# openai/baselines

Hardware: NVIDIA H100
Metric: PPO2 learner env-steps/sec (higher is better)
Workload: dtype f16 operands / f32 accumulate (GAE f64 carry)

## Files before the change

### baselines_b200/csrc/conv_shift.cu

```cuda
#include <stdlib.h>

#include <type_traits>

#include "common.cuh"
#include "tc_common.cuh"

namespace b200rl {

static constexpr int SH_BM = 128;
static constexpr int SH_CONSUMER_WARPS = 8;
static constexpr int SH_TMA_WARP = SH_CONSUMER_WARPS;
__host__ __device__ constexpr int sh_threads(bool u8) { return (SH_CONSUMER_WARPS + 1) * 32 + (u8 ? 256 : 0); }
static constexpr int SH_MAX_TAPS = 16;
__host__ __device__ constexpr int sh_arows(int KH) { return KH == 1 ? 160 : 144; }
__host__ __device__ constexpr int sh_stages(int KH) { return KH == 1 ? 6 : 4; }
static constexpr int SH_U8_STAGES = 12;
static constexpr int SH_U8_WRES_BYTES = 16 * 1024;
__host__ __device__ constexpr int sh_wgrad_krows(bool u8) { return u8 ? 128 : 64; }
__host__ __device__ constexpr int sh_wres_bytes(int KH, bool u8) {
  return u8 ? SH_U8_WRES_BYTES : KH == 1 ? 80 * 1024 : 64 * 1024;
}
static constexpr int SH_BAR_BYTES = 512;
__host__ __device__ constexpr int sh_mask_stage_bytes(int BN, bool DACT) { return DACT ? SH_BM * BN / 8 : 0; }
static constexpr int SH_EPI_WARP_BYTES = 16 * 64;
static constexpr int SH_EPI_BYTES = SH_CONSUMER_WARPS * SH_EPI_WARP_BYTES;
static constexpr int SH_WROWS_K = 96;
static constexpr int SH_WABYTES = SH_WROWS_K * 128;
__host__ __device__ constexpr int sh_wgrad_qw(int BN, int KH, bool u8) { return u8 ? 2 : BN == 32 ? 4 : KH == 1 ? 3 : 2; }

static constexpr int SH_ORDER_BAR = 2;
__device__ __forceinline__ void order_wait(int wg) {
  asm volatile("bar.sync %0, %1;" ::"r"(SH_ORDER_BAR + wg), "n"(SH_CONSUMER_WARPS * 32) : "memory");
}
__device__ __forceinline__ void order_pass(int wg) {
  asm volatile("bar.arrive %0, %1;" ::"r"(SH_ORDER_BAR + 1 - wg), "n"(SH_CONSUMER_WARPS * 32) : "memory");
}

struct AddrMap {
  int mode;
  long long sN, sY, sX;
  int Cq, s;
  int Cq_log2, s_log2;
};

__device__ __forceinline__ long long map_rowbase(const AddrMap& a, int n, int y, int x) {
  if (a.mode == 2) {
    const int sm = a.s - 1;
    return (long long)n * a.sN + (long long)(y >> a.s_log2) * a.sY + (long long)(x >> a.s_log2) * a.sX +
           ((((y & sm) << a.s_log2) + (x & sm)) << a.Cq_log2);
  }
  if (a.mode == 1) return (long long)n * a.sN + ((long long)y << a.s_log2) * a.sY + ((long long)x << a.s_log2) * a.sX;
  return (long long)n * a.sN + (long long)y * a.sY + (long long)x * a.sX;
}
__device__ __forceinline__ long long map_coloff(const AddrMap& a, int col) {
  if (a.mode == 1) {
    const int cls = col >> a.Cq_log2;
    return (long long)(cls >> a.s_log2) * a.sY + (long long)(cls & (a.s - 1)) * a.sX + (col & (a.Cq - 1));
  }
  return col;
}

struct FastDiv {
  uint32_t mul, sh, d;
  __device__ __forceinline__ uint32_t div(uint32_t n) const { return __umulhi(n, mul) >> sh; }
};
static FastDiv make_fastdiv(uint32_t d) {
  FastDiv f;
  f.d = d;
  uint32_t s = 0;
  while ((1ull << s) < d) ++s;
  if (s == 0) s = 1;
  f.mul = (uint32_t)(((1ull << (31 + s)) / d) + 1);
  f.sh = s - 1;
  return f;
}

struct U8Src {
  const uint8_t* x;
  const long long* idx;
  long long sample_bytes;
  int row_bytes;
  int y_bytes, x_bytes;
  FastDiv per, wg;
};

static constexpr int U8_WARPS = 8;

__device__ __forceinline__ void u8x16_to_f16(const uint4& q, uint4& lo, uint4& hi) {
  const uint32_t w[4] = {q.x, q.y, q.z, q.w};
  uint32_t o[8];
  const __half2 k1024 = __floats2half2_rn(1024.0f, 1024.0f);
#pragma unroll
  for (int i = 0; i < 4; ++i) {
    const uint32_t a = __byte_perm(w[i], 0x64646464u, 0x5140);
    const uint32_t b = __byte_perm(w[i], 0x64646464u, 0x5342);
    const __half2 ha = __hsub2(*reinterpret_cast<const __half2*>(&a), k1024);
    const __half2 hb = __hsub2(*reinterpret_cast<const __half2*>(&b), k1024);
    o[2 * i] = *reinterpret_cast<const uint32_t*>(&ha);
    o[2 * i + 1] = *reinterpret_cast<const uint32_t*>(&hb);
  }
  lo = make_uint4(o[0], o[1], o[2], o[3]);
  hi = make_uint4(o[4], o[5], o[6], o[7]);
}


__device__ __forceinline__ uint4 ldg_stream_v4(const void* p) {
  uint4 v;
  asm volatile("ld.global.nc.L1::no_allocate.v4.u32 {%0,%1,%2,%3}, [%4];"
               : "=r"(v.x), "=r"(v.y), "=r"(v.z), "=r"(v.w)
               : "l"(p));
  return v;
}
__device__ __forceinline__ void st_shared_v4(uint32_t addr, const uint4& v) {
  asm volatile("st.shared.v4.b32 [%0], {%1,%2,%3,%4};" ::"r"(addr), "r"(v.x), "r"(v.y), "r"(v.z), "r"(v.w) : "memory");
}

template <int TR, int STAGES>
struct U8Ring {
  static constexpr int UPT = TR / 32;
  static constexpr int ROWS = STAGES * TR + 32;
  static constexpr int BYTES = ROWS * 128;
  static_assert(TR % 32 == 0 && BYTES % 1024 == 0, "ring keeps the 1024 B swizzle atoms aligned");
};

__device__ __forceinline__ long long u8_lookup(const U8Src& u, long long row_start, int unit, int total, long long M,
                                               int lane) {
  const long long m = row_start + (long long)unit * 32 + lane;
  if (unit >= total || m < 0 || m >= M) return -1;
  const uint32_t n = u.per.div((uint32_t)m);
  return u.idx ? __ldg(u.idx + n) : (long long)n;
}
__device__ __forceinline__ void u8_load(const U8Src& u, long long row_start, int unit, long long sb, int lane,
                                        uint4 (&q)[4]) {
  if (sb >= 0) {
    const uint32_t mm = (uint32_t)(row_start + (long long)unit * 32 + lane);
    const uint32_t rem = mm - u.per.div(mm) * u.per.d;
    const uint32_t Y = u.wg.div(rem), X = rem - Y * u.wg.d;
    const uint8_t* src = u.x + sb * u.sample_bytes + (long long)(Y * (uint32_t)u.y_bytes + X * (uint32_t)u.x_bytes);
#pragma unroll
    for (int dy = 0; dy < 4; ++dy) q[dy] = ldg_stream_v4(src + (long long)dy * u.row_bytes);
  } else {
#pragma unroll
    for (int dy = 0; dy < 4; ++dy) q[dy] = make_uint4(0u, 0u, 0u, 0u);
  }
}

template <int TR, int STAGES, int D>
__device__ __forceinline__ void u8_ring_producer(const U8Src& u, long long M, long long row_start, int ntiles,
                                                 uint8_t* ring, uint64_t* full_bar, uint64_t* head_bar,
                                                 uint64_t* empty_bar, int pw, int lane) {
  using R = U8Ring<TR, STAGES>;
  constexpr int UPT = R::UPT, RND = U8_WARPS * D;
  if (ntiles <= 0) return;
  const int total = ntiles * UPT + 1;
  const uint32_t ring0 = smem_u32(ring) + lane * 128 + ((lane & 7) << 4);
  uint4 q[D][4];
  long long sb[D];
#pragma unroll
  for (int d = 0; d < D; ++d) sb[d] = u8_lookup(u, row_start, pw + U8_WARPS * d, total, M, lane);
#pragma unroll
  for (int d = 0; d < D; ++d) {
    u8_load(u, row_start, pw + U8_WARPS * d, sb[d], lane, q[d]);
    sb[d] = u8_lookup(u, row_start, pw + U8_WARPS * d + RND, total, M, lane);
  }
  for (int base = pw; base < total; base += RND) {
#pragma unroll
    for (int d = 0; d < D; ++d) {
      const int uc = base + U8_WARPS * d;
      if (uc < total) {
        const int tile = uc / UPT, ub = uc - tile * UPT;
        const int s = tile % STAGES;
        const uint32_t fill = (uint32_t)(tile / STAGES);
        mbar_wait(&empty_bar[s], (fill & 1u) ^ 1u);
        const uint32_t dst = ring0 + (uint32_t)(s * TR + ub * 32) * 128u;
        const bool mirror = (s == 0) && (ub == 0);
#pragma unroll
        for (int dy = 0; dy < 4; ++dy) {
          uint4 lo, hi;
          u8x16_to_f16(q[d][dy], lo, hi);
          st_shared_v4(dst ^ (uint32_t)((2 * dy) << 4), lo);
          st_shared_v4(dst ^ (uint32_t)((2 * dy + 1) << 4), hi);
// ... 148 lines not shown
    }
  } else if (U8 && warp > SH_TMA_WARP) {
    u8_ring_producer<SH_BM, STAGES, 2>(p.u8, p.M, (long long)tile_first * SH_BM + p.min_shift, tile_count, smem,
                                       full_bar, head_bar, empty_bar, warp - (SH_TMA_WARP + 1), lane);
  } else {
    const int wg = __shfl_sync(0xffffffffu, warp >> 2, 0), t = threadIdx.x & 127;
    const int row0 = PINGPONG ? 0 : wg * 64;
    const uint32_t w_base = smem_u32(wres);
    const float lo = (p.act == ACT_RELU) ? 0.0f : -INFINITY;
    const __half2 lo2 = __floats2half2_rn(lo, lo);
    const __half2 zero2 = __floats2half2_rn(0.0f, 0.0f);
    const int er = lane & 15, ep = lane >> 4;
    const int erow = row0 + 16 * (warp & 3) + er;
    uint32_t epi_addr[2];
#pragma unroll
    for (int jj = 0; jj < 2; ++jj)
      epi_addr[jj] = smem_u32(sepi + warp * SH_EPI_WARP_BYTES) + er * 64 + (((2 * jj + ep) ^ ((er >> 1) & 3)) << 4);
    const bool masked = DACT && p.saved_bits != nullptr;
    float acc[MH][BN / 2];
    mbar_wait(w_bar, 0);
    for (int i = PINGPONG ? wg : 0; i < tile_count; i += PINGPONG ? 2 : 1) {
      const int tile = tile_first + i * tile_stride;
      const int s = i % STAGES, s1 = (s + 1 == STAGES) ? 0 : s + 1;
      const uint32_t ph = (uint32_t)(i / STAGES) & 1u;
      mbar_wait(&full_bar[s], ph);
      if (U8) mbar_wait(&head_bar[s1], s1 == 0 ? ph ^ 1 : ph);
      if (PINGPONG && i > 0) order_wait(wg);
      const uint32_t a_base = smem_u32(smem + s * A_PITCH) + (uint32_t)(row0 * 128);
      wgmma_fence();
#pragma unroll 1
      for (int a = 0; a < p.taps; ++a) {
        const uint32_t at = a_base + (uint32_t)p.shift[a] * 128u;
        const uint32_t wt = w_base + (uint32_t)(a * KH * w_sub);
#pragma unroll
        for (int h = 0; h < KH; ++h) {
#pragma unroll
          for (int k = 0; k < 4; ++k) {
            const uint64_t bdesc = make_sdesc(wt + h * w_sub + k * 32, 16, 1024, 1);
#pragma unroll
            for (int mh = 0; mh < MH; ++mh) {
              const uint64_t adesc = make_sdesc(at + mh * 64 * 128 + h * SH_ABYTES + k * 32, 16, 1024, 1);
              wgmma_f16<BN, 0, 0>(acc[mh], adesc, bdesc, (a | h | k) ? 1u : 0u);
            }
          }
        }
      }
      wgmma_commit();
      if (PINGPONG && i + 1 < tile_count) order_pass(wg);
      wgmma_wait<0>();
      auto release = [&]() {
        __syncwarp();
        if (lane == 0) {
          mbar_arrive(&empty_bar[s]);
          if (U8) mbar_arrive(&empty_bar[s1]);
        }
      };
      uint32_t mrow[MH][BN / 32];
      if (masked) {
#pragma unroll
        for (int mh = 0; mh < MH; ++mh) {
          const uint32_t r = smem_u32(smask + s * MASK_STAGE) + (uint32_t)((erow + mh * 64) * (BN / 8));
#pragma unroll
          for (int i = 0; i < BN / 32; ++i) asm volatile("ld.shared.b32 %0, [%1];" : "=r"(mrow[mh][i]) : "r"(r + 4 * i));
        }
      } else {
        release();
      }

#pragma unroll
      for (int mh = 0; mh < MH; ++mh) {
        const uint32_t m = (uint32_t)tile * SH_BM + mh * 64 + erow;
        const uint32_t t2 = p.fwg.div(m);
        const int x = (int)(m - t2 * (uint32_t)p.Wg);
        const int n = (int)p.fhg.div(t2);
        const int y = (int)(t2 - (uint32_t)n * (uint32_t)p.Hg);
        const bool ok = ((long long)m < p.M) && (y < p.vy) && (x < p.vx);
        const long long obase = map_rowbase(p.omap, n, y, x);
#pragma unroll
        for (int ps = 0; ps < BN / 32; ++ps) {
#pragma unroll
          for (int jj = 0; jj < 2; ++jj) {
            const int b = 2 * (2 * ps + jj);
            uint32_t r[4];
#pragma unroll
            for (int k = 0; k < 4; ++k) {
              const int e = 4 * (b + (k >> 1)) + 2 * (k & 1);
              const int c = 8 * (b + (k >> 1)) + 2 * (t & 3);
              __half2 o;
              if (DACT) {
                o = __floats2half2_rn(acc[mh][e] * p.alpha, acc[mh][e + 1] * p.alpha);
              } else {
                o = __hmax2(__floats2half2_rn(fmaf(acc[mh][e], p.alpha, s_bias[c]),
                                              fmaf(acc[mh][e + 1], p.alpha, s_bias[c + 1])),
                            lo2);
              }
              r[k] = h2_bits(o);
            }
            stmatrix_x4(epi_addr[jj], r);
          }
          __syncwarp();
#pragma unroll
          for (int jj = 0; jj < 2; ++jj) {
            const int j = 2 * ps + jj;
            uint4 v = ld_shared_v4(epi_addr[jj]);
            const long long ocol = map_coloff(p.omap, 16 * j);
            if (masked) {
              const uint32_t b8 = (mrow[mh][j >> 1] >> (16 * (j & 1) + 8 * ep)) & 0xffu;
              v.x &= mask_pair(b8, 0);
              v.y &= mask_pair(b8, 1);
              v.z &= mask_pair(b8, 2);
              v.w &= mask_pair(b8, 3);
            }
            if (ok) st_global_v4(p.out + obase + ocol + 8 * ep, v);
            if (!DACT && p.bits_out != nullptr) {
              const uint32_t w[4] = {v.x, v.y, v.z, v.w};
              uint32_t bits = 0;
#pragma unroll
              for (int k = 0; k < 4; ++k) {
                const uint32_t gt = __hgt2_mask(*reinterpret_cast<const __half2*>(&w[k]), zero2);
                bits |= ((gt & 1u) | ((gt >> 15) & 2u)) << (2 * k);
              }
              bits <<= 8 * ep;
              bits |= __shfl_xor_sync(0xffffffffu, bits, 16);
              if (ok && ep == 0) p.bits_out[(obase + ocol) >> 4] = (uint16_t)bits;
            }
          }
          __syncwarp();
        }
      }
      if (masked) release();
    }
  }
}

struct ShiftWgradParams {
  U8Src u8;
  float* gbias;
  float alpha_b;
  long long M;
  int N;
  int taps;
  int kx;
  int shift[SH_MAX_TAPS];
  float* G;
  long long ldg;
  float alpha;
  int kb_total, kb_per_cta;
  float* ws_g;
  float* ws_b;
  long long grows;
};

template <int BN, int KH, bool U8>
__global__ void __launch_bounds__(sh_threads(U8), 1)
conv_shift_wgrad_kernel(const __grid_constant__ CUtensorMap tmX, const __grid_constant__ CUtensorMap tmD,
                        const __grid_constant__ ShiftWgradParams p) {
  constexpr int BROWB = (BN >= 64) ? 128 : BN * 2;
  constexpr uint32_t LAYOUT_B = sdesc_layout(BROWB);
  constexpr int KR = sh_wgrad_krows(U8);
  constexpr int B_BYTES = KR * BROWB;
  constexpr int B_REGION = (B_BYTES + 1023) & ~1023;
  constexpr int STAGES = (KH == 1) ? 8 : 6;
  constexpr int QW = sh_wgrad_qw(BN, KH, U8);
  static_assert(!U8 || KH == 1, "the uint8-fed layer has 64 space-to-depth channels");
  using Ring = U8Ring<KR, STAGES>;
  constexpr int A_PITCH = U8 ? KR * 128 : KH * SH_WABYTES + B_REGION;
  constexpr int B_PITCH = U8 ? B_REGION : KH * SH_WABYTES + B_REGION;
  constexpr int B_BASE = U8 ? Ring::BYTES : KH * SH_WABYTES;
  constexpr int SMEM_TILES = U8 ? Ring::BYTES + STAGES * B_REGION : STAGES * (KH * SH_WABYTES + B_REGION);
  extern __shared__ uint8_t smem_raw[];
  uint8_t* smem = reinterpret_cast<uint8_t*>((reinterpret_cast<uintptr_t>(smem_raw) + 1023) & ~uintptr_t(1023));
  uint64_t* bars = reinterpret_cast<uint64_t*>(smem + SMEM_TILES);
  uint64_t* full_bar = bars;
  uint64_t* empty_bar = bars + STAGES;
  uint64_t* head_bar = bars + 2 * STAGES;

  const int warp = threadIdx.x >> 5, lane = threadIdx.x & 31;
  const int kb0 = blockIdx.x * p.kb_per_cta;
  const int kb1 = min(kb0 + p.kb_per_cta, p.kb_total);
  const int nchunks = p.taps * p.kx * KH;
  const uint32_t ncta = U8 ? 1u : cluster_nctarank();

  if (threadIdx.x == 0) {
    for (int s = 0; s < STAGES; ++s) {
      mbar_init(&full_bar[s], U8 ? 1 + Ring::UPT : 1);
      mbar_init(&empty_bar[s], SH_CONSUMER_WARPS * ncta);
      if (U8) mbar_init(&head_bar[s], 1);
    }
    fence_barrier_init();
  }
  if (ncta > 1) cluster_sync();
  else __syncthreads();

  if (warp == SH_TMA_WARP) {
    if (elect_one()) {
      tma_prefetch_desc(&tmX);
      tma_prefetch_desc(&tmD);
    }
    __syncwarp();
    const uint32_t rank = U8 ? 0u : cluster_ctarank();
    const uint16_t mask = (uint16_t)((1u << ncta) - 1u);
    int s = 0;
    uint32_t ph = 0;
    for (int kb = kb0; kb < kb1; ++kb) {
      mbar_wait(&empty_bar[s], ph ^ 1);
      if (elect_one()) {
        uint8_t* sa = smem + s * A_PITCH;
        uint8_t* sb = smem + B_BASE + s * B_PITCH;
        mbar_arrive_expect_tx(&full_bar[s], (uint32_t)((U8 ? 0 : KH * SH_WABYTES) + B_BYTES));
        if (U8) {
          tma_load_2d(sb, &tmD, &full_bar[s], 0, kb * KR);
        } else {
          for (int b = (int)rank; b <= KH; b += (int)ncta) {
            void* dst = b < KH ? (void*)(sa + b * SH_WABYTES) : (void*)sb;
            const CUtensorMap* tm = b < KH ? &tmX : &tmD;
            if (ncta == 1) tma_load_2d(dst, tm, &full_bar[s], b < KH ? b * 64 : 0, kb * KR);
            else tma_load_2d_multicast(dst, tm, &full_bar[s], b < KH ? b * 64 : 0, kb * KR, mask);
          }
        }
      }
      __syncwarp();
      if (++s == STAGES) { s = 0; ph ^= 1; }
    }
  } else if (U8 && warp > SH_TMA_WARP) {
    u8_ring_producer<KR, STAGES, 3>(p.u8, p.M, (long long)kb0 * KR, kb1 - kb0, smem, full_bar, head_bar, empty_bar,
                                    warp - (SH_TMA_WARP + 1), lane);
  } else {
    const int wg = warp >> 2, t = threadIdx.x & 127;
    const int nwg = 2 * (int)gridDim.y, w = 2 * (int)blockIdx.y + wg;
    const int q0 = w * (nchunks / nwg) + min(w, nchunks % nwg);
    const int nq = nchunks / nwg + (w < nchunks % nwg ? 1 : 0);
    int a_rel[QW];
#pragma unroll
    for (int i = 0; i < QW; ++i) {
      const int q = min(q0 + i, nchunks - 1);
      const int tap = q / KH, h = q - tap * KH;
      a_rel[i] = h * SH_WABYTES + (p.shift[tap / p.kx] + tap % p.kx) * 128;
    }
    const bool do_bias = p.gbias != nullptr && blockIdx.y == 0;
    constexpr int LPR = BROWB / 8;
    constexpr int RG = 32 / LPR;
    const int cq = lane % LPR, rg = lane / LPR;
    const int chunk = (cq * 8) >> 4, within = (cq * 8) & 15;
    float bsum[4] = {0.f, 0.f, 0.f, 0.f};
    auto bias_sums = [&](int st) {
      const uint8_t* sb = smem + B_BASE + st * B_PITCH;
#pragma unroll 4
      for (int r = warp * RG + rg; r < KR; r += SH_CONSUMER_WARPS * RG) {
        const int sw = (BROWB == 128) ? (r & 7) : ((r >> 1) & 3);
        const uint2 v = *reinterpret_cast<const uint2*>(sb + r * BROWB + ((chunk ^ sw) << 4) + within);
        bsum[0] += __half2float(__ushort_as_half((unsigned short)(v.x & 0xffffu)));
        bsum[1] += __half2float(__ushort_as_half((unsigned short)(v.x >> 16)));
        bsum[2] += __half2float(__ushort_as_half((unsigned short)(v.y & 0xffffu)));
        bsum[3] += __half2float(__ushort_as_half((unsigned short)(v.y >> 16)));
      }
    };
    auto release = [&](int st) {
      __syncwarp();
      if (U8 || ncta == 1) {
        if (lane == 0) mbar_arrive(&empty_bar[st]);
      } else if (lane < (int)ncta) {
        mbar_arrive_cluster(&empty_bar[st], (uint32_t)lane);
      }
    };
    constexpr int NP = (QW + 2) * (BN / 2) <= 128 ? 2 : 1;
    float acc[QW][BN / 2], part[NP][BN / 2];
#pragma unroll
    for (int i = 0; i < QW; ++i)
#pragma unroll
      for (int e = 0; e < BN / 2; ++e) acc[i][e] = 0.0f;
    auto add_part = [&](float(&a)[BN / 2], const float(&pt)[BN / 2]) {
#pragma unroll
      for (int e = 0; e < BN / 2; ++e) a[e] += pt[e];
    };
    auto consume = [&](auto nq_c) {
      constexpr int NQ = decltype(nq_c)::value;
      int s = 0;
      uint32_t ph = 0;
      for (int kb = kb0; kb < kb1; ++kb) {
        const int s1 = (s + 1 == STAGES) ? 0 : s + 1;
        mbar_wait(&full_bar[s], ph);
        if (U8) mbar_wait(&head_bar[s1], s1 == 0 ? ph ^ 1 : ph);
        const uint32_t a_base = smem_u32(smem + s * A_PITCH);
        const uint32_t b_base = smem_u32(smem + B_BASE + s * B_PITCH);
        if (NQ == 0 && do_bias) bias_sums(s);
#pragma unroll
        for (int i = 0; i < NQ; ++i) {
          wgmma_fence();
#pragma unroll
          for (int k = 0; k < KR / 16; ++k) {
            const uint64_t adesc = make_sdesc(a_base + a_rel[i] + k * 16 * 128, 8 * 1024, 1024, 1);
            const uint64_t bdesc = make_sdesc(b_base + k * 16 * BROWB, 8 * 8 * BROWB, 8 * BROWB, LAYOUT_B);
            wgmma_f16<BN, 1, 1>(part[i % NP], adesc, bdesc, k > 0 ? 1u : 0u);
          }
          wgmma_commit();
          if (i == 0 && do_bias) bias_sums(s);
          wgmma_wait<NP - 1>();
          if (i >= NP - 1) add_part(acc[i - (NP - 1)], part[(i - (NP - 1)) % NP]);
        }
        if constexpr (NP == 2 && NQ > 0) {
          wgmma_wait<0>();
          add_part(acc[NQ - 1], part[(NQ - 1) % NP]);
        }
        release(s);
        s = s1;
        if (s == 0) ph ^= 1;
      }
    };
    static_assert(QW >= 2 && QW <= 4, "conv_shift_wgrad: 2..4 chunks per warpgroup");
    switch (nq) {
      case 0: consume(std::integral_constant<int, 0>{}); break;
      case 1: consume(std::integral_constant<int, 1>{}); break;
      case 2: consume(std::integral_constant<int, 2>{}); break;
      default:
        if constexpr (QW >= 3) if (nq == 3) consume(std::integral_constant<int, 3>{});
        if constexpr (QW >= 4) if (nq == 4) consume(std::integral_constant<int, 4>{});
    }
    if (do_bias) {
      __shared__ float s_bsum[SH_CONSUMER_WARPS][64];
#pragma unroll
      for (int o = LPR; o < 32; o <<= 1)
#pragma unroll
        for (int i = 0; i < 4; ++i) bsum[i] += __shfl_xor_sync(0xffffffffu, bsum[i], o);
      if (rg == 0) {
#pragma unroll
        for (int i = 0; i < 4; ++i) s_bsum[warp][4 * cq + i] = bsum[i];
      }
      asm volatile("bar.sync 1, %0;" ::"n"(SH_CONSUMER_WARPS * 32) : "memory");
      if ((int)threadIdx.x < p.N) {
        float b = 0.0f;
#pragma unroll
        for (int w = 0; w < SH_CONSUMER_WARPS; ++w) b += s_bsum[w][threadIdx.x];
        p.ws_b[(long long)blockIdx.x * p.N + threadIdx.x] = b * p.alpha_b;
      }
    }
    if (kb1 > kb0) {
#pragma unroll
      for (int i = 0; i < QW; ++i) {
        if (i < nq) {
#pragma unroll
          for (int e = 0; e < BN / 2; ++e) {
            const int cn = acc_col(t, e);
            const long long grow = (long long)(q0 + i) * 64 + acc_row(t, e);
            if (cn < p.N) p.ws_g[((long long)blockIdx.x * p.grows + grow) * p.N + cn] = acc[i][e] * p.alpha;
          }
        }
      }
    }
  }
  if (ncta > 1) cluster_sync();
}

static U8Src make_u8src(const void* x, const long long* idx, int H, int W, int C, int s) {
  U8Src u{};
  u.x = reinterpret_cast<const uint8_t*>(x);
  if (!x) return u;
  u.idx = idx;
  u.sample_bytes = (long long)H * W * C;
  u.row_bytes = W * C;
  u.y_bytes = s * W * C;
  u.x_bytes = s * C;
  u.per = make_fastdiv((uint32_t)((H / s) * (W / s)));
  u.wg = make_fastdiv((uint32_t)(W / s));
  return u;
}

template <int BN, int KH, bool DACT, bool U8 = false>
static int launch_fwd(const CUtensorMap& tmX, const CUtensorMap& tmW, const ShiftParams& p, cudaStream_t st) {
  constexpr int STAGES = U8 ? SH_U8_STAGES : sh_stages(KH);
  constexpr int SMEM = (U8 ? U8Ring<SH_BM, STAGES>::BYTES : STAGES * KH * sh_arows(KH) * 128) + sh_wres_bytes(KH, U8) +
                       1024 + SH_BAR_BYTES + STAGES * sh_mask_stage_bytes(BN, DACT) + SH_EPI_BYTES;
  static_assert(SMEM + 1024 <= 227 * 1024, "conv_shift_fwd: shared memory budget (+ static bias array)");
  static bool attr = false;
  auto kern = conv_shift_fwd_kernel<BN, KH, DACT, U8>;
  if (!attr) {
    cudaError_t e = cudaFuncSetAttribute(kern, cudaFuncAttributeMaxDynamicSharedMemorySize, SMEM);
    if (e != cudaSuccess) {
      set_last_error("conv_shift_fwd: smem attr %d: %s", SMEM, cudaGetErrorString(e));
      return B200RL_ERR_CUDA;
    }
    attr = true;
  }
  const int grid = p.num_tiles < device_num_sms() ? p.num_tiles : device_num_sms();
  kern<<<grid, sh_threads(U8), SMEM, st>>>(tmX, tmW, p);
  return check_launch("conv_shift_fwd_kernel");
}

static int wgrad_cluster(int groups) {
  int g = groups < 8 ? groups : 8;
  while (groups % g) --g;
  return g;
}

template <int BN, int KH, bool U8 = false>
static int launch_wgrad(const CUtensorMap& tmX, const CUtensorMap& tmD, const ShiftWgradParams& p, dim3 grid,
                        cudaStream_t st) {
  constexpr int STAGES = (KH == 1) ? 8 : 6;
  constexpr int KR = sh_wgrad_krows(U8);
  constexpr int BROWB = (BN >= 64) ? 128 : BN * 2;
  constexpr int B_REGION = (KR * BROWB + 1023) & ~1023;
  constexpr int SMEM =
      (U8 ? U8Ring<KR, STAGES>::BYTES + STAGES * B_REGION : STAGES * (KH * SH_WABYTES + B_REGION)) + 1024 + 512;
  static_assert(SMEM <= 227 * 1024, "conv_shift_wgrad: shared memory budget");
  static bool attr = false;
  static int co_resident[9] = {};
  auto kern = conv_shift_wgrad_kernel<BN, KH, U8>;
  if (!attr) {
    cudaError_t e = cudaFuncSetAttribute(kern, cudaFuncAttributeMaxDynamicSharedMemorySize, SMEM);
    if (e != cudaSuccess) {
      set_last_error("conv_shift_wgrad: smem attr %d: %s", SMEM, cudaGetErrorString(e));
      return B200RL_ERR_CUDA;
    }
    attr = true;
  }
  int g = U8 ? 1 : wgrad_cluster((int)grid.y);
  cudaLaunchAttribute cl;
  cl.id = cudaLaunchAttributeClusterDimension;
  cl.val.clusterDim.x = 1;
  cl.val.clusterDim.y = (unsigned)g;
  cl.val.clusterDim.z = 1;
  cudaLaunchConfig_t cfg = {};
  cfg.gridDim = grid;
  cfg.blockDim = dim3(sh_threads(U8));
  cfg.dynamicSmemBytes = SMEM;
  cfg.stream = st;
  cfg.attrs = &cl;
  cfg.numAttrs = 1;
  if (g > 1) {
    if (co_resident[g] == 0) {
      cudaError_t e = cudaOccupancyMaxActiveClusters(&co_resident[g], kern, &cfg);
      if (e != cudaSuccess) {
        set_last_error("conv_shift_wgrad: cluster occupancy (%d CTAs): %s", g, cudaGetErrorString(e));
        co_resident[g] = 0;
        return B200RL_ERR_CUDA;
      }
    }
    if (co_resident[g] * g < device_num_sms()) g = 1;
  }
  cfg.numAttrs = g > 1 ? 1 : 0;
  const cudaError_t e = cudaLaunchKernelEx(&cfg, kern, tmX, tmD, p);
  const int rc = check_launch("conv_shift_wgrad_kernel");
  if (rc == B200RL_OK && e != cudaSuccess) {
    set_last_error("conv_shift_wgrad_kernel: %s", cudaGetErrorString(e));
    return B200RL_ERR_CUDA;
  }
  return rc;
}

static int ilog2(int v) { int l = 0; while ((1 << l) < v) ++l; return l; }
static bool fill_map(AddrMap& a, const long long* m) {
  a.mode = (int)m[0]; a.sN = m[1]; a.sY = m[2]; a.sX = m[3]; a.Cq = (int)m[4]; a.s = (int)m[5];
  a.Cq_log2 = a.s_log2 = 0;
  if (a.mode == 0) return true;
  if (a.Cq < 16 || (a.Cq & (a.Cq - 1)) || a.s < 1 || (a.s & (a.s - 1))) return false;
  a.Cq_log2 = ilog2(a.Cq); a.s_log2 = ilog2(a.s);
  return true;
}

}

using namespace b200rl;

extern "C" int b200rl_conv_shift_fwd(const void* X, long long B, int Hg, int Wg, int C, const void* W, long long ldw,
                                     int N, int taps, const int* shifts, int vy, int vx, void* out,
                                     const long long* omap, const long long* smap, const float* bias, int act, int dact,
                                     float alpha, const void* u8_x, const long long* u8_idx, int u8_H, int u8_W,
                                     int u8_C, int u8_s, void* bits_out, const void* saved_bits, void* stream_) {
  cudaStream_t stream = static_cast<cudaStream_t>(stream_);
  B200RL_REQUIRE((X || u8_x) && W && out && omap && B > 0, "conv_shift_fwd: null operand");
  B200RL_REQUIRE(!(bits_out && dact) && !(saved_bits && !(dact && smap)), "conv_shift_fwd: bits_out is a forward output, saved_bits a dact input (with smap)");
  if (u8_x) {
    B200RL_REQUIRE(C == 64 && u8_s * u8_C == 16 && u8_s == 4 && u8_H == Hg * u8_s && u8_W == Wg * u8_s && !dact &&
                       N == 32 && (reinterpret_cast<uintptr_t>(u8_x) & 15) == 0 && (u8_W * u8_C) % 16 == 0,
                   "conv_shift_fwd: fused uint8 source needs s=4, s*C=16, N=32, 16 B aligned rows");
  }
  B200RL_REQUIRE(C == 64 || C == 128, "conv_shift_fwd: C must be 64 or 128 (got %d)", C);
  B200RL_REQUIRE(N == 32 || N == 64 || N == 128, "conv_shift_fwd: N must be 32, 64 or 128 (got %d)", N);
  B200RL_REQUIRE(taps >= 1 && taps <= SH_MAX_TAPS, "conv_shift_fwd: 1..%d taps", SH_MAX_TAPS);
  B200RL_REQUIRE((C == 64 || C == 128) && (long long)taps * (C / 64) * N * 128 <= sh_wres_bytes(C / 64, u8_x != nullptr),
                 "conv_shift_fwd: weights do not fit in smem");
  ShiftParams p = {};
  int lo = shifts[0], hi = shifts[0];
  for (int t = 1; t < taps; ++t) { lo = shifts[t] < lo ? shifts[t] : lo; hi = shifts[t] > hi ? shifts[t] : hi; }
  B200RL_REQUIRE(hi - lo <= sh_arows(C / 64) - SH_BM, "conv_shift_fwd: shift span %d too large for C = %d", hi - lo,
                 C);
  B200RL_REQUIRE(B * Hg * Wg < (1LL << 31) - 4096, "conv_shift_fwd: too many rows");
  p.M = B * Hg * Wg; p.Hg = Hg; p.Wg = Wg; p.N = N; p.taps = taps; p.min_shift = lo;
  for (int t = 0; t < taps; ++t) p.shift[t] = shifts[t] - lo;
  p.vy = vy; p.vx = vx; p.out = reinterpret_cast<__half*>(out);
  B200RL_REQUIRE(fill_map(p.omap, omap), "conv_shift_fwd: output map needs power-of-two Cq >= 16 and s");
  p.bits_out = reinterpret_cast<uint16_t*>(bits_out);
  p.saved_bits = reinterpret_cast<const uint16_t*>(saved_bits);
  B200RL_REQUIRE(((omap[1] | omap[2] | omap[3]) & 15) == 0 && (reinterpret_cast<uintptr_t>(out) & 31) == 0,
                 "conv_shift_fwd: output strides must be multiples of 16 elements, base 32-byte aligned");
  if (saved_bits)
    B200RL_REQUIRE(smap[0] == 0 && smap[3] == N && smap[2] == (long long)Wg * N && smap[1] == (long long)Hg * Wg * N &&
                       (reinterpret_cast<uintptr_t>(saved_bits) & 15) == 0,
                   "conv_shift_fwd: saved_bits needs the row-contiguous map (0, Hg*Wg*N, Wg*N, N) and a 16-byte aligned "
                   "base");
  p.bias = bias; p.act = act; p.dact = dact; p.alpha = alpha;
  p.num_tiles = (int)((p.M + SH_BM - 1) / SH_BM);
  p.u8 = make_u8src(u8_x, u8_idx, u8_H, u8_W, u8_C, u8_s);
  B200RL_REQUIRE(Hg >= 2 && Wg >= 2, "conv_shift_fwd: grid must be at least 2x2");
  p.fwg = make_fastdiv((uint32_t)Wg);
  p.fhg = make_fastdiv((uint32_t)Hg);
  CUtensorMap tmX, tmW;
  int rc;
  B200RL_REQUIRE(act == ACT_NONE || act == ACT_RELU, "conv_shift_fwd: activation must be none or relu");
  if ((rc = make_tmap_2d_f16(&tmW, W, N, (long long)taps * C, ldw, 64, N)) != 0) return rc;
  if (u8_x) {
    B200RL_REQUIRE(hi - lo <= 32, "conv_shift_fwd: uint8-fed shift span %d exceeds one 32-row unit", hi - lo);
    return launch_fwd<32, 1, false, true>(tmW, tmW, p, stream);
  }
  if ((rc = make_tmap_2d_f16(&tmX, X, p.M, C, C, 64, sh_arows(C / 64))) != 0) return rc;
  const int KH = C / 64;
#define SHIFT_FWD_CASE(bn)                                                                                    \
  if (N == bn) {                                                                                              \
    if (dact) return KH == 1 ? launch_fwd<bn, 1, true>(tmX, tmW, p, stream) : launch_fwd<bn, 2, true>(tmX, tmW, p, stream); \
    return KH == 1 ? launch_fwd<bn, 1, false>(tmX, tmW, p, stream) : launch_fwd<bn, 2, false>(tmX, tmW, p, stream);        \
  }
  SHIFT_FWD_CASE(32)
  SHIFT_FWD_CASE(64)
  SHIFT_FWD_CASE(128)
#undef SHIFT_FWD_CASE
  return B200RL_ERR_UNSUPPORTED;
}

extern "C" int b200rl_conv_shift_wgrad(const void* X, long long rows, int C, const void* dY, int N, int taps,
                                       const int* shifts, float* G, long long ldg, float alpha, float* gbias,
                                       float alpha_b, int max_ctas, const void* u8_x, const long long* u8_idx, int u8_H,
                                       int u8_W, int u8_C, int u8_s, int kx, void* stream_) {
  cudaStream_t stream = static_cast<cudaStream_t>(stream_);
  B200RL_REQUIRE((X || u8_x) && dY && G && rows > 0, "conv_shift_wgrad: null operand");
  if (kx < 1) kx = 1;
  B200RL_REQUIRE(kx <= 3, "conv_shift_wgrad: kx must be 1..3");
  if (u8_x)
    B200RL_REQUIRE(C == 64 && u8_s == 4 && u8_s * u8_C == 16 && N == 32 && u8_H % 4 == 0 && u8_W % 4 == 0 &&
                       (reinterpret_cast<uintptr_t>(u8_x) & 15) == 0,
                   "conv_shift_wgrad: fused uint8 source needs s=4, s*C=16, N=32");
  B200RL_REQUIRE(C == 64 || C == 128, "conv_shift_wgrad: C must be 64 or 128");
  B200RL_REQUIRE(N == 32 || N == 64, "conv_shift_wgrad: N must be 32 or 64 (got %d)", N);
  B200RL_REQUIRE(taps >= 1 && taps <= SH_MAX_TAPS, "conv_shift_wgrad: 1..%d taps", SH_MAX_TAPS);
  const int KH = C / 64;
  ShiftWgradParams p = {};
  for (int t = 0; t < taps; ++t) {
    B200RL_REQUIRE(shifts[t] >= 0 && shifts[t] + kx - 1 <= SH_WROWS_K - 64, "conv_shift_wgrad: shift %d out of range",
                   shifts[t]);
    p.shift[t] = shifts[t];
  }
  p.M = rows; p.N = N; p.taps = taps; p.kx = kx; p.G = G; p.ldg = ldg; p.alpha = alpha;
  p.gbias = gbias; p.alpha_b = alpha_b;
  const int KR = sh_wgrad_krows(u8_x != nullptr);
  p.kb_total = (int)((rows + KR - 1) / KR);
  int ctas = device_num_sms();
  if (max_ctas > 0 && max_ctas < ctas) ctas = max_ctas;
  if (ctas > p.kb_total) ctas = p.kb_total;
  p.kb_per_cta = (p.kb_total + ctas - 1) / ctas;
  const int qw = sh_wgrad_qw(N, KH, u8_x != nullptr);
  const dim3 grid((p.kb_total + p.kb_per_cta - 1) / p.kb_per_cta, (taps * kx * KH + 2 * qw - 1) / (2 * qw));
  p.u8 = make_u8src(u8_x, u8_idx, u8_H, u8_W, u8_C, u8_s);
  p.grows = (long long)taps * kx * KH * 64;
  const size_t g_floats = (size_t)grid.x * p.grows * N;
  float* ws = det_workspace(g_floats + (size_t)grid.x * N, stream);
  if (!ws) return B200RL_ERR_CUDA;
  p.ws_g = ws;
  p.ws_b = ws + g_floats;
  CUtensorMap tmX, tmD;
  int rc;
  if ((rc = make_tmap_2d_f16(&tmD, dY, rows, N, N, N < 64 ? N : 64, KR)) != 0) return rc;
  if (u8_x) {
    rc = launch_wgrad<32, 1, true>(tmD, tmD, p, grid, stream);
  } else {
    if ((rc = make_tmap_2d_f16(&tmX, X, rows, C, C, 64, SH_WROWS_K)) != 0) return rc;
    if (N == 32) rc = KH == 1 ? launch_wgrad<32, 1>(tmX, tmD, p, grid, stream) : launch_wgrad<32, 2>(tmX, tmD, p, grid, stream);
    else rc = KH == 1 ? launch_wgrad<64, 1>(tmX, tmD, p, grid, stream) : launch_wgrad<64, 2>(tmX, tmD, p, grid, stream);
  }
// ... 5 lines not shown
```

### baselines_b200/csrc/tc_common.cuh

```cuda
#pragma once
#include "common.cuh"
#include "wgmma.cuh"

namespace b200rl {

enum : int { MODE_F16_ACT = 0, MODE_F32_STORE = 1, MODE_F32_ATOMIC = 2, MODE_F16_DACT = 3, MODE_F16_SHUFFLE = 4 };
enum : int { ACT_NONE = 0, ACT_RELU = 1, ACT_TANH = 2 };

__host__ __device__ constexpr uint32_t sdesc_layout(int row_bytes) {
  return row_bytes == 128 ? 1u : row_bytes == 64 ? 2u : 3u;
}
__device__ __forceinline__ uint64_t make_sdesc(uint32_t saddr, uint32_t lbo_bytes, uint32_t sbo_bytes, uint32_t layout) {
  uint64_t d = 0;
  d |= (uint64_t)((saddr & 0x3FFFFu) >> 4);
  d |= (uint64_t)((lbo_bytes >> 4) & 0x3FFFu) << 16;
  d |= (uint64_t)((sbo_bytes >> 4) & 0x3FFFu) << 32;
  d |= (uint64_t)layout << 62;
  return d;
}

__device__ __forceinline__ int acc_row(int t, int e) { return 16 * (t >> 5) + ((t & 31) >> 2) + 8 * ((e >> 1) & 1); }
__device__ __forceinline__ int acc_col(int t, int e) { return 8 * (e >> 2) + 2 * (t & 3) + (e & 1); }

__device__ __forceinline__ void tma_load_im2col_4d(void* smem_dst, const CUtensorMap* tmap, uint64_t* bar, int c, int w,
                                                   int h, int n, uint16_t off_w, uint16_t off_h) {
  asm volatile(
      "cp.async.bulk.tensor.4d.shared::cluster.global.im2col.mbarrier::complete_tx::bytes"
      " [%0], [%1, {%3, %4, %5, %6}], [%2], {%7, %8};"
      ::"r"(smem_u32(smem_dst)), "l"(tmap), "r"(smem_u32(bar)), "r"(c), "r"(w), "r"(h), "r"(n), "h"(off_w), "h"(off_h)
      : "memory");
}

__device__ __forceinline__ float apply_act(float x, int act) {
  if (act == ACT_RELU) return fmaxf(x, 0.0f);
  if (act == ACT_TANH) return tanhf(x);
  return x;
}
__device__ __forceinline__ float act_grad_from_saved(float h, int act) {
  if (act == ACT_RELU) return h > 0.0f ? 1.0f : 0.0f;
  if (act == ACT_TANH) return 1.0f - h * h;
  return 1.0f;
}

int make_tmap_2d_f16(CUtensorMap* tm, const void* ptr, long long rows, long long cols, long long ld, int box_cols,
                     int box_rows);

}
```

### baselines_b200/csrc/wgmma.cuh

```cuda
#pragma once
#include <stdint.h>

namespace b200rl {

template <int TA, int TB>
__device__ __forceinline__ void wgmma_f16_n32(float (&d)[16], uint64_t da, uint64_t db, uint32_t scale_d) {
  asm volatile(
      "{\n\t.reg .pred p;\n\tsetp.ne.b32 p, %18, 0;\n\t"
      "wgmma.mma_async.sync.aligned.m64n32k16.f32.f16.f16 {%0, %1, %2, %3, %4, %5, %6, %7, %8, %9, %10, %11, %12, %13, %14, %15}, %16, %17, p, 1, 1, %19, %20;\n\t}"
      : "+f"(d[0]), "+f"(d[1]), "+f"(d[2]), "+f"(d[3]), "+f"(d[4]), "+f"(d[5]), "+f"(d[6]), "+f"(d[7]),
        "+f"(d[8]), "+f"(d[9]), "+f"(d[10]), "+f"(d[11]), "+f"(d[12]), "+f"(d[13]), "+f"(d[14]), "+f"(d[15])
      : "l"(da), "l"(db), "r"(scale_d), "n"(TA), "n"(TB));
}

template <int TA, int TB>
__device__ __forceinline__ void wgmma_f16_n64(float (&d)[32], uint64_t da, uint64_t db, uint32_t scale_d) {
  asm volatile(
      "{\n\t.reg .pred p;\n\tsetp.ne.b32 p, %34, 0;\n\t"
      "wgmma.mma_async.sync.aligned.m64n64k16.f32.f16.f16 {%0, %1, %2, %3, %4, %5, %6, %7, %8, %9, %10, %11, %12, %13, %14, %15, %16, %17, %18, %19, %20, %21, %22, %23, %24, %25, %26, %27, %28, %29, %30, %31}, %32, %33, p, 1, 1, %35, %36;\n\t}"
      : "+f"(d[0]), "+f"(d[1]), "+f"(d[2]), "+f"(d[3]), "+f"(d[4]), "+f"(d[5]), "+f"(d[6]), "+f"(d[7]),
        "+f"(d[8]), "+f"(d[9]), "+f"(d[10]), "+f"(d[11]), "+f"(d[12]), "+f"(d[13]), "+f"(d[14]), "+f"(d[15]),
        "+f"(d[16]), "+f"(d[17]), "+f"(d[18]), "+f"(d[19]), "+f"(d[20]), "+f"(d[21]), "+f"(d[22]), "+f"(d[23]),
        "+f"(d[24]), "+f"(d[25]), "+f"(d[26]), "+f"(d[27]), "+f"(d[28]), "+f"(d[29]), "+f"(d[30]), "+f"(d[31])
      : "l"(da), "l"(db), "r"(scale_d), "n"(TA), "n"(TB));
}

template <int TA, int TB>
__device__ __forceinline__ void wgmma_f16_n128(float (&d)[64], uint64_t da, uint64_t db, uint32_t scale_d) {
  asm volatile(
      "{\n\t.reg .pred p;\n\tsetp.ne.b32 p, %66, 0;\n\t"
      "wgmma.mma_async.sync.aligned.m64n128k16.f32.f16.f16 {%0, %1, %2, %3, %4, %5, %6, %7, %8, %9, %10, %11, %12, %13, %14, %15, %16, %17, %18, %19, %20, %21, %22, %23, %24, %25, %26, %27, %28, %29, %30, %31, %32, %33, %34, %35, %36, %37, %38, %39, %40, %41, %42, %43, %44, %45, %46, %47, %48, %49, %50, %51, %52, %53, %54, %55, %56, %57, %58, %59, %60, %61, %62, %63}, %64, %65, p, 1, 1, %67, %68;\n\t}"
      : "+f"(d[0]), "+f"(d[1]), "+f"(d[2]), "+f"(d[3]), "+f"(d[4]), "+f"(d[5]), "+f"(d[6]), "+f"(d[7]),
        "+f"(d[8]), "+f"(d[9]), "+f"(d[10]), "+f"(d[11]), "+f"(d[12]), "+f"(d[13]), "+f"(d[14]), "+f"(d[15]),
        "+f"(d[16]), "+f"(d[17]), "+f"(d[18]), "+f"(d[19]), "+f"(d[20]), "+f"(d[21]), "+f"(d[22]), "+f"(d[23]),
        "+f"(d[24]), "+f"(d[25]), "+f"(d[26]), "+f"(d[27]), "+f"(d[28]), "+f"(d[29]), "+f"(d[30]), "+f"(d[31]),
        "+f"(d[32]), "+f"(d[33]), "+f"(d[34]), "+f"(d[35]), "+f"(d[36]), "+f"(d[37]), "+f"(d[38]), "+f"(d[39]),
        "+f"(d[40]), "+f"(d[41]), "+f"(d[42]), "+f"(d[43]), "+f"(d[44]), "+f"(d[45]), "+f"(d[46]), "+f"(d[47]),
        "+f"(d[48]), "+f"(d[49]), "+f"(d[50]), "+f"(d[51]), "+f"(d[52]), "+f"(d[53]), "+f"(d[54]), "+f"(d[55]),
        "+f"(d[56]), "+f"(d[57]), "+f"(d[58]), "+f"(d[59]), "+f"(d[60]), "+f"(d[61]), "+f"(d[62]), "+f"(d[63])
      : "l"(da), "l"(db), "r"(scale_d), "n"(TA), "n"(TB));
}

template <int TA, int TB>
__device__ __forceinline__ void wgmma_f16_n256(float (&d)[128], uint64_t da, uint64_t db, uint32_t scale_d) {
  asm volatile(
      "{\n\t.reg .pred p;\n\tsetp.ne.b32 p, %130, 0;\n\t"
      "wgmma.mma_async.sync.aligned.m64n256k16.f32.f16.f16 {%0, %1, %2, %3, %4, %5, %6, %7, %8, %9, %10, %11, %12, %13, %14, %15, %16, %17, %18, %19, %20, %21, %22, %23, %24, %25, %26, %27, %28, %29, %30, %31, %32, %33, %34, %35, %36, %37, %38, %39, %40, %41, %42, %43, %44, %45, %46, %47, %48, %49, %50, %51, %52, %53, %54, %55, %56, %57, %58, %59, %60, %61, %62, %63, %64, %65, %66, %67, %68, %69, %70, %71, %72, %73, %74, %75, %76, %77, %78, %79, %80, %81, %82, %83, %84, %85, %86, %87, %88, %89, %90, %91, %92, %93, %94, %95, %96, %97, %98, %99, %100, %101, %102, %103, %104, %105, %106, %107, %108, %109, %110, %111, %112, %113, %114, %115, %116, %117, %118, %119, %120, %121, %122, %123, %124, %125, %126, %127}, %128, %129, p, 1, 1, %131, %132;\n\t}"
      : "+f"(d[0]), "+f"(d[1]), "+f"(d[2]), "+f"(d[3]), "+f"(d[4]), "+f"(d[5]), "+f"(d[6]), "+f"(d[7]),
        "+f"(d[8]), "+f"(d[9]), "+f"(d[10]), "+f"(d[11]), "+f"(d[12]), "+f"(d[13]), "+f"(d[14]), "+f"(d[15]),
        "+f"(d[16]), "+f"(d[17]), "+f"(d[18]), "+f"(d[19]), "+f"(d[20]), "+f"(d[21]), "+f"(d[22]), "+f"(d[23]),
        "+f"(d[24]), "+f"(d[25]), "+f"(d[26]), "+f"(d[27]), "+f"(d[28]), "+f"(d[29]), "+f"(d[30]), "+f"(d[31]),
        "+f"(d[32]), "+f"(d[33]), "+f"(d[34]), "+f"(d[35]), "+f"(d[36]), "+f"(d[37]), "+f"(d[38]), "+f"(d[39]),
        "+f"(d[40]), "+f"(d[41]), "+f"(d[42]), "+f"(d[43]), "+f"(d[44]), "+f"(d[45]), "+f"(d[46]), "+f"(d[47]),
        "+f"(d[48]), "+f"(d[49]), "+f"(d[50]), "+f"(d[51]), "+f"(d[52]), "+f"(d[53]), "+f"(d[54]), "+f"(d[55]),
        "+f"(d[56]), "+f"(d[57]), "+f"(d[58]), "+f"(d[59]), "+f"(d[60]), "+f"(d[61]), "+f"(d[62]), "+f"(d[63]),
        "+f"(d[64]), "+f"(d[65]), "+f"(d[66]), "+f"(d[67]), "+f"(d[68]), "+f"(d[69]), "+f"(d[70]), "+f"(d[71]),
        "+f"(d[72]), "+f"(d[73]), "+f"(d[74]), "+f"(d[75]), "+f"(d[76]), "+f"(d[77]), "+f"(d[78]), "+f"(d[79]),
        "+f"(d[80]), "+f"(d[81]), "+f"(d[82]), "+f"(d[83]), "+f"(d[84]), "+f"(d[85]), "+f"(d[86]), "+f"(d[87]),
        "+f"(d[88]), "+f"(d[89]), "+f"(d[90]), "+f"(d[91]), "+f"(d[92]), "+f"(d[93]), "+f"(d[94]), "+f"(d[95]),
        "+f"(d[96]), "+f"(d[97]), "+f"(d[98]), "+f"(d[99]), "+f"(d[100]), "+f"(d[101]), "+f"(d[102]), "+f"(d[103]),
        "+f"(d[104]), "+f"(d[105]), "+f"(d[106]), "+f"(d[107]), "+f"(d[108]), "+f"(d[109]), "+f"(d[110]), "+f"(d[111]),
        "+f"(d[112]), "+f"(d[113]), "+f"(d[114]), "+f"(d[115]), "+f"(d[116]), "+f"(d[117]), "+f"(d[118]), "+f"(d[119]),
        "+f"(d[120]), "+f"(d[121]), "+f"(d[122]), "+f"(d[123]), "+f"(d[124]), "+f"(d[125]), "+f"(d[126]), "+f"(d[127])
      : "l"(da), "l"(db), "r"(scale_d), "n"(TA), "n"(TB));
}

template <int N, int TA, int TB>
__device__ __forceinline__ void wgmma_f16(float (&d)[N / 2], uint64_t da, uint64_t db, uint32_t scale_d) {
  if constexpr (N == 32) wgmma_f16_n32<TA, TB>(d, da, db, scale_d);
  if constexpr (N == 64) wgmma_f16_n64<TA, TB>(d, da, db, scale_d);
  if constexpr (N == 128) wgmma_f16_n128<TA, TB>(d, da, db, scale_d);
  if constexpr (N == 256) wgmma_f16_n256<TA, TB>(d, da, db, scale_d);
}

}
```

Measured before the change: 1.198 million.

## Use register-sourced WGMMA and setmaxnreg split in shift-conv wgrad kernel

For the non-uint8 wgrad kernel with BN=64, the gradient tile is loaded once per stage into registers via ldmatrix.trans and used as the register-sourced A operand of WGMMA. The activation tiles become the shared-memory B operand, which swaps the accumulator row and column mapping in the epilogue. The block grows to 12 warps so setmaxnreg can take registers from the producer warps and give them to the consumers. That allows more chunks per warpgroup (QW 2→4 for KH>1) and an always double-buffered partial. The aim is less repeated shared-memory B traffic and more accumulator reuse per stage, at the cost of higher register pressure and possible spills.

```diff
diff --git a/baselines_b200/csrc/conv_shift.cu b/baselines_b200/csrc/conv_shift.cu
--- a/baselines_b200/csrc/conv_shift.cu
+++ b/baselines_b200/csrc/conv_shift.cu
@@ -26,7 +26,10 @@
 static constexpr int SH_EPI_BYTES = SH_CONSUMER_WARPS * SH_EPI_WARP_BYTES;
 static constexpr int SH_WROWS_K = 96;
 static constexpr int SH_WABYTES = SH_WROWS_K * 128;
-__host__ __device__ constexpr int sh_wgrad_qw(int BN, int KH, bool u8) { return u8 ? 2 : BN == 32 ? 4 : KH == 1 ? 3 : 2; }
+__host__ __device__ constexpr int sh_wgrad_qw(int BN, int KH, bool u8) { return u8 ? 2 : BN == 32 ? 4 : KH == 1 ? 3 : 4; }
+__host__ __device__ constexpr int sh_wgrad_threads(bool u8) { return u8 ? sh_threads(true) : (SH_CONSUMER_WARPS + 4) * 32; }
+static constexpr int SH_WGRAD_PRODUCER_REGS = 40, SH_WGRAD_CONSUMER_REGS = 232;
+static_assert(128 * SH_WGRAD_PRODUCER_REGS + 256 * SH_WGRAD_CONSUMER_REGS <= 65536, "wgrad register split");
 
 static constexpr int SH_ORDER_BAR = 2;
 __device__ __forceinline__ void order_wait(int wg) {
@@ -481,7 +484,7 @@
 };
 
 template <int BN, int KH, bool U8>
-__global__ void __launch_bounds__(sh_threads(U8), 1)
+__global__ void __launch_bounds__(sh_wgrad_threads(U8), 1)
 conv_shift_wgrad_kernel(const __grid_constant__ CUtensorMap tmX, const __grid_constant__ CUtensorMap tmD,
                         const __grid_constant__ ShiftWgradParams p) {
   constexpr int BROWB = (BN >= 64) ? 128 : BN * 2;
@@ -520,42 +523,45 @@
   }
   if (ncta > 1) cluster_sync();
   else __syncthreads();
-
-  if (warp == SH_TMA_WARP) {
-    if (elect_one()) {
-      tma_prefetch_desc(&tmX);
-      tma_prefetch_desc(&tmD);
-    }
-    __syncwarp();
-    const uint32_t rank = U8 ? 0u : cluster_ctarank();
-    const uint16_t mask = (uint16_t)((1u << ncta) - 1u);
-    int s = 0;
-    uint32_t ph = 0;
-    for (int kb = kb0; kb < kb1; ++kb) {
-      mbar_wait(&empty_bar[s], ph ^ 1);
+  if (warp >= SH_TMA_WARP) {
+    if constexpr (!U8) setmaxnreg_dec<SH_WGRAD_PRODUCER_REGS>();
+    if (warp == SH_TMA_WARP) {
       if (elect_one()) {
-        uint8_t* sa = smem + s * A_PITCH;
-        uint8_t* sb = smem + B_BASE + s * B_PITCH;
-        mbar_arrive_expect_tx(&full_bar[s], (uint32_t)((U8 ? 0 : KH * SH_WABYTES) + B_BYTES));
-        if (U8) {
-          tma_load_2d(sb, &tmD, &full_bar[s], 0, kb * KR);
-        } else {
-          for (int b = (int)rank; b <= KH; b += (int)ncta) {
-            void* dst = b < KH ? (void*)(sa + b * SH_WABYTES) : (void*)sb;
-            const CUtensorMap* tm = b < KH ? &tmX : &tmD;
-            if (ncta == 1) tma_load_2d(dst, tm, &full_bar[s], b < KH ? b * 64 : 0, kb * KR);
-            else tma_load_2d_multicast(dst, tm, &full_bar[s], b < KH ? b * 64 : 0, kb * KR, mask);
+        tma_prefetch_desc(&tmX);
+        tma_prefetch_desc(&tmD);
+      }
+      __syncwarp();
+      const uint32_t rank = U8 ? 0u : cluster_ctarank();
+      const uint16_t mask = (uint16_t)((1u << ncta) - 1u);
+      int s = 0;
+      uint32_t ph = 0;
+      for (int kb = kb0; kb < kb1; ++kb) {
+        mbar_wait(&empty_bar[s], ph ^ 1);
+        if (elect_one()) {
+          uint8_t* sa = smem + s * A_PITCH;
+          uint8_t* sb = smem + B_BASE + s * B_PITCH;
+          mbar_arrive_expect_tx(&full_bar[s], (uint32_t)((U8 ? 0 : KH * SH_WABYTES) + B_BYTES));
+          if (U8) {
+            tma_load_2d(sb, &tmD, &full_bar[s], 0, kb * KR);
+          } else {
+            for (int b = (int)rank; b <= KH; b += (int)ncta) {
+              void* dst = b < KH ? (void*)(sa + b * SH_WABYTES) : (void*)sb;
+              const CUtensorMap* tm = b < KH ? &tmX : &tmD;
+              if (ncta == 1) tma_load_2d(dst, tm, &full_bar[s], b < KH ? b * 64 : 0, kb * KR);
+              else tma_load_2d_multicast(dst, tm, &full_bar[s], b < KH ? b * 64 : 0, kb * KR, mask);
+            }
           }
         }
-      }
-      __syncwarp();
-      if (++s == STAGES) { s = 0; ph ^= 1; }
-    }
-  } else if (U8 && warp > SH_TMA_WARP) {
-    u8_ring_producer<KR, STAGES, 3>(p.u8, p.M, (long long)kb0 * KR, kb1 - kb0, smem, full_bar, head_bar, empty_bar,
-                                    warp - (SH_TMA_WARP + 1), lane);
+        __syncwarp();
+        if (++s == STAGES) { s = 0; ph ^= 1; }
+      }
+    } else if constexpr (U8) {
+      u8_ring_producer<KR, STAGES, 3>(p.u8, p.M, (long long)kb0 * KR, kb1 - kb0, smem, full_bar, head_bar, empty_bar,
+                                      warp - (SH_TMA_WARP + 1), lane);
+    }
   } else {
-    const int wg = warp >> 2, t = threadIdx.x & 127;
+    if constexpr (!U8) setmaxnreg_inc<SH_WGRAD_CONSUMER_REGS>();
+    const int wg = __shfl_sync(0xffffffffu, warp >> 2, 0), t = threadIdx.x & 127;
     const int nwg = 2 * (int)gridDim.y, w = 2 * (int)blockIdx.y + wg;
     const int q0 = w * (nchunks / nwg) + min(w, nchunks % nwg);
     const int nq = nchunks / nwg + (w < nchunks % nwg ? 1 : 0);
@@ -592,8 +598,7 @@
         mbar_arrive_cluster(&empty_bar[st], (uint32_t)lane);
       }
     };
-    constexpr int NP = (QW + 2) * (BN / 2) <= 128 ? 2 : 1;
-    float acc[QW][BN / 2], part[NP][BN / 2];
+    float acc[QW][BN / 2], part[2][BN / 2];
 #pragma unroll
     for (int i = 0; i < QW; ++i)
 #pragma unroll
@@ -602,6 +607,11 @@
 #pragma unroll
       for (int e = 0; e < BN / 2; ++e) a[e] += pt[e];
     };
+    constexpr bool RS = !U8 && BN == 64;
+    constexpr int KS = KR / 16;
+    uint32_t frag[KS][4];
+    const uint32_t frag_off = (uint32_t)((8 * (lane >> 4) + (lane & 7)) * 128 +
+                                         (((2 * (warp & 3) + ((lane >> 3) & 1)) ^ (lane & 7)) << 4));
     auto consume = [&](auto nq_c) {
       constexpr int NQ = decltype(nq_c)::value;
       int s = 0;
@@ -613,23 +623,30 @@
         const uint32_t a_base = smem_u32(smem + s * A_PITCH);
         const uint32_t b_base = smem_u32(smem + B_BASE + s * B_PITCH);
         if (NQ == 0 && do_bias) bias_sums(s);
+        if constexpr (RS && NQ > 0)
+#pragma unroll
+          for (int k = 0; k < KS; ++k) ldmatrix_x4_trans(frag[k], b_base + k * 16 * 128 + frag_off);
 #pragma unroll
         for (int i = 0; i < NQ; ++i) {
           wgmma_fence();
 #pragma unroll
-          for (int k = 0; k < KR / 16; ++k) {
-            const uint64_t adesc = make_sdesc(a_base + a_rel[i] + k * 16 * 128, 8 * 1024, 1024, 1);
-            const uint64_t bdesc = make_sdesc(b_base + k * 16 * BROWB, 8 * 8 * BROWB, 8 * BROWB, LAYOUT_B);
-            wgmma_f16<BN, 1, 1>(part[i % NP], adesc, bdesc, k > 0 ? 1u : 0u);
+          for (int k = 0; k < KS; ++k) {
+            const uint64_t xdesc = make_sdesc(a_base + a_rel[i] + k * 16 * 128, 8 * 1024, 1024, 1);
+            if constexpr (RS) {
+              wgmma_f16_rs<BN, 1>(part[i % 2], frag[k], xdesc, k > 0 ? 1u : 0u);
+            } else {
+              const uint64_t bdesc = make_sdesc(b_base + k * 16 * BROWB, 8 * 8 * BROWB, 8 * BROWB, LAYOUT_B);
+              wgmma_f16<BN, 1, 1>(part[i % 2], xdesc, bdesc, k > 0 ? 1u : 0u);
+            }
           }
           wgmma_commit();
           if (i == 0 && do_bias) bias_sums(s);
-          wgmma_wait<NP - 1>();
-          if (i >= NP - 1) add_part(acc[i - (NP - 1)], part[(i - (NP - 1)) % NP]);
-        }
-        if constexpr (NP == 2 && NQ > 0) {
+          wgmma_wait<1>();
+          if (i >= 1) add_part(acc[i - 1], part[(i - 1) % 2]);
+        }
+        if constexpr (NQ > 0) {
           wgmma_wait<0>();
-          add_part(acc[NQ - 1], part[(NQ - 1) % NP]);
+          add_part(acc[NQ - 1], part[(NQ - 1) % 2]);
         }
         release(s);
         s = s1;
@@ -669,8 +686,8 @@
         if (i < nq) {
 #pragma unroll
           for (int e = 0; e < BN / 2; ++e) {
-            const int cn = acc_col(t, e);
-            const long long grow = (long long)(q0 + i) * 64 + acc_row(t, e);
+            const int cn = RS ? acc_row(t, e) : acc_col(t, e);
+            const long long grow = (long long)(q0 + i) * 64 + (RS ? acc_col(t, e) : acc_row(t, e));
             if (cn < p.N) p.ws_g[((long long)blockIdx.x * p.grows + grow) * p.N + cn] = acc[i][e] * p.alpha;
           }
         }
@@ -750,7 +767,7 @@
   cl.val.clusterDim.z = 1;
   cudaLaunchConfig_t cfg = {};
   cfg.gridDim = grid;
-  cfg.blockDim = dim3(sh_threads(U8));
+  cfg.blockDim = dim3(sh_wgrad_threads(U8));
   cfg.dynamicSmemBytes = SMEM;
   cfg.stream = st;
   cfg.attrs = &cl;
diff --git a/baselines_b200/csrc/tc_common.cuh b/baselines_b200/csrc/tc_common.cuh
--- a/baselines_b200/csrc/tc_common.cuh
+++ b/baselines_b200/csrc/tc_common.cuh
@@ -21,6 +21,18 @@
 
 __device__ __forceinline__ int acc_row(int t, int e) { return 16 * (t >> 5) + ((t & 31) >> 2) + 8 * ((e >> 1) & 1); }
 __device__ __forceinline__ int acc_col(int t, int e) { return 8 * (e >> 2) + 2 * (t & 3) + (e & 1); }
+
+template <int REGS>
+__device__ __forceinline__ void setmaxnreg_dec() { asm volatile("setmaxnreg.dec.sync.aligned.u32 %0;" ::"n"(REGS)); }
+template <int REGS>
+__device__ __forceinline__ void setmaxnreg_inc() { asm volatile("setmaxnreg.inc.sync.aligned.u32 %0;" ::"n"(REGS)); }
+
+__device__ __forceinline__ void ldmatrix_x4_trans(uint32_t (&r)[4], uint32_t addr) {
+  asm volatile("ldmatrix.sync.aligned.m8n8.x4.trans.shared.b16 {%0, %1, %2, %3}, [%4];"
+               : "=r"(r[0]), "=r"(r[1]), "=r"(r[2]), "=r"(r[3])
+               : "r"(addr)
+               : "memory");
+}
 
 __device__ __forceinline__ void tma_load_im2col_4d(void* smem_dst, const CUtensorMap* tmap, uint64_t* bar, int c, int w,
                                                    int h, int n, uint16_t off_w, uint16_t off_h) {
diff --git a/baselines_b200/csrc/wgmma.cuh b/baselines_b200/csrc/wgmma.cuh
--- a/baselines_b200/csrc/wgmma.cuh
+++ b/baselines_b200/csrc/wgmma.cuh
@@ -73,4 +73,21 @@
   if constexpr (N == 256) wgmma_f16_n256<TA, TB>(d, da, db, scale_d);
 }
 
+template <int TB>
+__device__ __forceinline__ void wgmma_f16_rs_n64(float (&d)[32], const uint32_t (&a)[4], uint64_t db, uint32_t scale_d) {
+  asm volatile(
+      "{\n\t.reg .pred p;\n\tsetp.ne.b32 p, %37, 0;\n\t"
+      "wgmma.mma_async.sync.aligned.m64n64k16.f32.f16.f16 {%0, %1, %2, %3, %4, %5, %6, %7, %8, %9, %10, %11, %12, %13, %14, %15, %16, %17, %18, %19, %20, %21, %22, %23, %24, %25, %26, %27, %28, %29, %30, %31}, {%32, %33, %34, %35}, %36, p, 1, 1, %38;\n\t}"
+      : "+f"(d[0]), "+f"(d[1]), "+f"(d[2]), "+f"(d[3]), "+f"(d[4]), "+f"(d[5]), "+f"(d[6]), "+f"(d[7]),
+        "+f"(d[8]), "+f"(d[9]), "+f"(d[10]), "+f"(d[11]), "+f"(d[12]), "+f"(d[13]), "+f"(d[14]), "+f"(d[15]),
+        "+f"(d[16]), "+f"(d[17]), "+f"(d[18]), "+f"(d[19]), "+f"(d[20]), "+f"(d[21]), "+f"(d[22]), "+f"(d[23]),
+        "+f"(d[24]), "+f"(d[25]), "+f"(d[26]), "+f"(d[27]), "+f"(d[28]), "+f"(d[29]), "+f"(d[30]), "+f"(d[31])
+      : "r"(a[0]), "r"(a[1]), "r"(a[2]), "r"(a[3]), "l"(db), "r"(scale_d), "n"(TB));
 }
+
+template <int N, int TB>
+__device__ __forceinline__ void wgmma_f16_rs(float (&d)[N / 2], const uint32_t (&a)[4], uint64_t db, uint32_t scale_d) {
+  if constexpr (N == 64) wgmma_f16_rs_n64<TB>(d, a, db, scale_d);
+}
+
+}
```

Result: faster. 1.235 million (median of 6 runs) (+3.1%).
